# netsniff-ng/netsniff-ng

Hardware: AMD Instinct MI355X
Metric: Mpkt/s + GB/s device-resident dissect, 64B & IMIX; bit-exact fields vs ref (higher is better)
Workload: dtype u8

## Files before the change

netsniff-ng_amd/csrc/nsd_internal.h:

```cpp
#ifndef NSD_INTERNAL_H
#define NSD_INTERNAL_H

#include <hip/hip_runtime_api.h>
#include <stddef.h>
#include <stdint.h>
#include <stdio.h>

#include <string>
#include <vector>

#include "../../include/netsniff_dissect.h"

#define NSD_HIDDEN __attribute__((visibility("hidden")))

NSD_HIDDEN inline bool hip_ok(hipError_t e, const char *what)
{
	if (e != hipSuccess) {
		fprintf(stderr, "netsniff-dissect: %s: %s\n", what, hipGetErrorString(e));
		return false;
	}
	return true;
}

template <class T>
NSD_HIDDEN inline bool grow(T *&p, size_t &cap, size_t need)
{
	if (need <= cap)
		return true;
	if (p)
		(void)hipFree(p);
	p = nullptr;
	cap = 0;
	const size_t want = need + need / 4 + 64;
	if (!hip_ok(hipMalloc(&p, want * sizeof(T)), "hipMalloc"))
		return false;
	cap = want;
	return true;
}

inline size_t batch_extent(const nsd_desc_t *desc, size_t n)
{
	size_t used = 0;
	for (size_t j = 0; j < n; j++) {
		const size_t e = NSD_DESC_OFF(desc[j]) + NSD_DESC_CAPLEN(desc[j]);
		used = e > used ? e : used;
	}
	return used;
}

extern "C" int nsd_launch_dissect_rec(const uint8_t *d_frames, const uint64_t *d_desc, const void *d_sll,
				      uint32_t n, int start_id, int mode, void *d_rec, int compact, uint32_t *d_ext,
				      uint32_t ext_words, uint32_t *d_ext_used, uint64_t *d_counters, void *d_ws,
				      int grid, hipStream_t stream);
extern "C" int nsd_launch_dissect(const uint8_t *d_frames, const uint64_t *d_desc, uint32_t n, int start_id,
				  int mode, nsd_rec *d_rec, uint32_t *d_ext, uint32_t ext_words, uint32_t *d_ext_used,
				  uint64_t *d_counters, void *d_ws, int grid, hipStream_t stream);
extern "C" int nsd_launch_dissect_sll(const uint8_t *d_frames, const uint64_t *d_desc, const void *d_sll,
				      uint32_t n, int start_id, int mode, nsd_rec *d_rec, uint32_t *d_ext,
				      uint32_t ext_words, uint32_t *d_ext_used, uint64_t *d_counters, void *d_ws,
				      int grid, hipStream_t stream);
extern "C" size_t nsd_launch_workspace_bytes(uint32_t n);

NSD_HIDDEN int nsd_start_for(int linktype);
extern "C" NSD_HIDDEN int nsd_pipe_retarget(nsd_pipe *p, int linktype, int mode);

extern "C" NSD_HIDDEN long nsd_flow_feed_host(nsd_flow_table *t, const uint8_t *frames, size_t frames_len,
					      const nsd_desc_t *desc, const nsd_sll_t *sll, uint32_t n, int linktype,
					      int mode, const nsd_bpf_prog *filter, const uint64_t *ts, uint64_t *ts_max,
					      uint64_t base);
extern "C" NSD_HIDDEN int nsd_flow_feed_records(nsd_flow_table *t, const uint8_t *frames, size_t frames_len,
						const nsd_desc_t *desc, uint32_t n, const nsd_rec *rec,
						const uint32_t *ext, uint32_t ext_words, const uint64_t *ts, uint64_t base);
NSD_HIDDEN long nsd_flow_expire_rows(nsd_flow_table *t, uint64_t before, uint32_t flags, uint32_t max,
				     std::vector<nsd_flow> &rows, uint64_t *stats);
NSD_HIDDEN long nsd_flow_expire_rows_ts(nsd_flow_table *t, uint64_t before_ns, uint32_t flags, uint32_t max,
					std::vector<nsd_flowt> &rows, uint64_t *stats);

extern "C" NSD_HIDDEN void nsd_if_cache_reset(void);
extern "C" NSD_HIDDEN void nsd_replay_release(void);
extern "C" NSD_HIDDEN void nsd_device_ctx_release(void);

namespace nsd {
bool render_layer(std::string &s, const uint8_t *pkt, uint32_t caplen, int id, uint32_t start, uint32_t tail,
		  int mode, uint16_t ip_csum, bool icmp_bad, const nsd_sll_t *sll, uint32_t &data,
		  uint32_t &ntail, bool &next);
void render_hex(std::string &s, const uint8_t *pkt, uint32_t caplen, uint32_t from, uint32_t len);
void render_ascii(std::string &s, const uint8_t *pkt, uint32_t caplen, uint32_t from, uint32_t len);
void format_frame_hdr(std::string &s, const nsd_frame_hdr_t &fh, const nsd_sll_t *sll, const uint8_t *pkt,
		      uint32_t caplen, int linktype, int mode, uint64_t count);
int render_packet_cpu(std::string &text, const uint8_t *packet, size_t len, int linktype, int mode,
		      const nsd_sll_t *sll);
int format_replay_part(std::string &s, const uint8_t *frames, const nsd_desc_t *desc, const nsd_frame_hdr_t *fh,
		       const nsd_sll_t *sll, const nsd_crec *rec, const uint32_t *ext, uint64_t count0, uint32_t lo,
		       uint32_t hi, int linktype, int mode);
int cpu_step(int mode, const uint8_t *pkt, uint32_t caplen, int id, uint32_t &data, uint32_t &tail,
	     uint16_t &ip_csum, uint8_t &flags, const nsd_sll_t *sll);
void cpu_count_packet(const uint8_t *pkt, uint32_t caplen, int linktype, int mode, const nsd_sll_t *sll,
		      uint64_t *counters);
}

#endif
```

netsniff-ng_amd/csrc/nsd_kernels.hip:

```cpp
#include <hip/hip_runtime.h>
#include <stdint.h>
#include <string.h>

#include <atomic>
#include <mutex>

#include "nsd_internal.h"
#include "nsd_walk.h"

namespace nsd {

constexpr int BLOCK = 256;
constexpr int WAVES = BLOCK / 64;

#ifndef NSD_WIN2
#define NSD_WIN2 128
#endif
#ifndef NSD_CSUM_U
#define NSD_CSUM_U 12
#endif
#ifndef NSD_FAST_CSUM_U
#define NSD_FAST_CSUM_U 8
#endif
#ifndef NSD_CSUM_LANES
#define NSD_CSUM_LANES 8
#endif
#ifndef NSD_MINW
#define NSD_MINW 4
#endif
#ifndef NSD_FAST_MINW
#define NSD_FAST_MINW 4
#endif
#ifndef NSD_FAST_MINW_FULL
#define NSD_FAST_MINW_FULL 4
#endif
#ifndef NSD_FAST_BPC
#define NSD_FAST_BPC 3
#endif
#ifndef NSD_FAST_BPC_SMALL
#define NSD_FAST_BPC_SMALL 2
#endif
#ifndef NSD_GROUP_BLOCKS
#define NSD_GROUP_BLOCKS 4u
#endif
#ifndef NSD_L2PF
#define NSD_L2PF 16
#endif
#ifndef NSD_REFILL
#define NSD_REFILL 16
#endif
#ifndef NSD_WIN_AHEAD
#define NSD_WIN_AHEAD 32
#endif
#ifndef NSD_SCHED_SAMPLE
#define NSD_SCHED_SAMPLE 32
#endif
#ifndef NSD_SMALL_FRAME
#define NSD_SMALL_FRAME 128
#endif

constexpr int WIN1 = 64;
constexpr int WIN2 = NSD_WIN2;
constexpr int row_of(int W) { return W / 4 + 4; }

typedef uint32_t v4u __attribute__((ext_vector_type(4)));
typedef __attribute__((address_space(1))) const v4u gv4u;
__device__ __forceinline__ uint32_t lanes_below(uint64_t m)
{
	return __builtin_amdgcn_mbcnt_hi((uint32_t)(m >> 32), __builtin_amdgcn_mbcnt_lo((uint32_t)m, 0));
}

__device__ __forceinline__ uint64_t wave_sum64(uint64_t v)
{
#pragma unroll
	for (int o = 32; o > 0; o >>= 1)
		v += __shfl_xor(v, o, 64);
	return v;
}

struct HbmBytes {
	const uint8_t *p;
	uint32_t caplen;
	__device__ __forceinline__ uint8_t b(uint32_t o) const { return o < caplen ? p[o] : 0; }
	__device__ __forceinline__ uint16_t be16(uint32_t o) const { return (uint16_t)(b(o) << 8 | b(o + 1)); }
};

template <bool FAST, int WIN>
struct LSrc {
	const uint32_t *win;
	const uint8_t *lay3t;
	const uint32_t *stept;
	const uint8_t *p;
	uint32_t caplen;
	uint32_t m;
	uint32_t wb;
	mutable bool miss;
	uint32_t sw;
	uint32_t wl = WIN;

	__device__ __forceinline__ uint32_t dw(uint32_t j) const { return win[j ^ sw]; }
	__device__ __forceinline__ int lay3(uint32_t key) const { return lay3t[key & 255]; }
	__device__ __forceinline__ uint32_t step(int id) const { return stept[id & 31]; }
	__device__ __forceinline__ uint32_t l2h(uint32_t h) const { return stept[32 + (h & 31)]; }
	__device__ __forceinline__ uint32_t dword_at(uint32_t o) const
	{
		const uint32_t r = o + m - wb;
		uint32_t j = r >> 2;
		j = j > WIN / 4 - 1 ? WIN / 4 - 1 : j;
		const uint32_t v = __builtin_amdgcn_alignbyte(dw(j + 1), dw(j), r & 3);
		if constexpr (FAST)
			return o >= caplen ? 0u : v;
		return v;
	}
	__device__ __forceinline__ bool missed() const { return miss; }
	__device__ __forceinline__ uint8_t b(uint32_t o) const
	{
		const uint32_t r = o + m - wb;
		if constexpr (FAST) {
			if (r < WIN)
				return (uint8_t)(dw(r >> 2) >> ((r & 3) * 8));
			if (o < caplen)
				miss = true;
			return 0;
		} else {
			if (o >= caplen)
				return 0;
			return r < wl ? (uint8_t)(dw(r >> 2) >> ((r & 3) * 8)) : p[o];
		}
	}
	__device__ __forceinline__ uint16_t le16(uint32_t o) const
	{
		const uint32_t r = o + m - wb;
		if (r + 1 < wl && (r & 3) != 3 && (FAST || o + 2 <= caplen))
			return (uint16_t)(dw(r >> 2) >> ((r & 3) * 8));
		return (uint16_t)(b(o) | b(o + 1) << 8);
	}
	__device__ __forceinline__ uint16_t be16(uint32_t o) const
	{
// ... 1108 lines not shown
constexpr int FROW = WIN1 / 4;

struct FastShared {
	alignas(16) uint32_t win[WAVES][64 * FROW];
	unsigned long long cnt[NSD_NCOUNTERS];
	uint32_t ops[32];
	uint8_t lay3[256];
	uint32_t pcnt[WAVES];
};

__device__ __forceinline__ void stage_write_sw(uint32_t *wwin, const Chunks<WIN1> &ch, int lane)
{
#pragma unroll
	for (int r = 0; r < 4; r++) {
		const int t = r * 64 + lane;
		const int q = t / 4, c = t % 4;
		const uint32_t nv = (ch.nv >> (8 * r)) & 0xFF;
		uint32_t w[4] = { ch.v[r].x, ch.v[r].y, ch.v[r].z, ch.v[r].w };
		if (nv < 16) {
#pragma unroll
			for (int j = 0; j < 4; j++) {
				const uint32_t bp = 4 * j;
				if (bp >= nv)
					w[j] = 0;
				else if (bp + 4 > nv)
					w[j] &= (1u << ((nv - bp) * 8)) - 1u;
			}
		}
		*(uint4 *)(wwin + q * FROW + ((c ^ swz_of((uint32_t)q, 4)) << 2)) = make_uint4(w[0], w[1], w[2], w[3]);
	}
}

__device__ __forceinline__ uint32_t fold_weighted(uint32_t sum, bool odd)
{
	sum = (sum >> 16) + (sum & 0xFFFF);
	sum = (sum >> 16) + (sum & 0xFFFF);
	return odd ? ((sum & 0xFF) << 8 | sum >> 8) : sum;
}

static_assert(k_plain_lay3[6] == NSD_OPS_TCP && k_plain_lay3[17] == NSD_OPS_UDP,
	      "plain_walk's protocol map differs from eth_lay3");

__device__ __forceinline__ bool plain_is(const LSrc<true, WIN1> &s, uint32_t caplen)
{
	const uint32_t r = s.m + 12, j = r >> 2, sh = r & 3;
	const uint32_t d12 = __builtin_amdgcn_alignbyte(s.dw(j + 1), s.dw(j), sh);
	const uint32_t d20 = __builtin_amdgcn_alignbyte(s.dw(j + 3), s.dw(j + 2), sh);
	const uint32_t proto = d20 >> 24;
	return caplen >= 42 && (d12 & 0xFFFFFFu) == 0x450008u && (proto == 6 || proto == 17);
}

__device__ __forceinline__ void plain_walk(const LSrc<true, WIN1> &s, uint32_t caplen, WalkOut &w)
{
	const uint32_t r = s.m + 12, j = r >> 2, sh = r & 3;
	const uint32_t w0 = s.dw(j), w1 = s.dw(j + 1), w2 = s.dw(j + 2), w3 = s.dw(j + 3), w4 = s.dw(j + 4),
		       w5 = s.dw(j + 5), w6 = s.dw(j + 6);
	const uint32_t d12 = __builtin_amdgcn_alignbyte(w1, w0, sh), d16 = __builtin_amdgcn_alignbyte(w2, w1, sh),
		       d20 = __builtin_amdgcn_alignbyte(w3, w2, sh), d24 = __builtin_amdgcn_alignbyte(w4, w3, sh),
		       d28 = __builtin_amdgcn_alignbyte(w5, w4, sh), d32 = __builtin_amdgcn_alignbyte(w6, w5, sh);
	uint32_t sum = (d12 >> 16) + (d32 & 0xFFFF);
	sum = __builtin_amdgcn_sad_u16(d16, 0u, sum);
	sum = __builtin_amdgcn_sad_u16(d20, 0u, sum);
	sum = __builtin_amdgcn_sad_u16(d24, 0u, sum);
	sum = __builtin_amdgcn_sad_u16(d28, 0u, sum);
	sum = (sum >> 16) + (sum & 0xffff);
	sum += sum >> 16;
	w.ip_csum = (uint16_t)~sum;
	const int32_t x = (int32_t)__builtin_bswap16((uint16_t)d16) - 20;
	if (x >= 0 && (uint32_t)x < caplen - 34)
		w.tail = 34 + (uint32_t)x;
	const bool tcp = (d20 >> 24) == 6;
	const int l4 = tcp ? NSD_OPS_TCP : NSD_OPS_UDP;
	w.chain = NSD_OPS_ETHERNET | NSD_OPS_IPV4 << 5 | (uint32_t)l4 << 10;
	w.offA = (uint64_t)14 << 16 | (uint64_t)34 << 32;
	w.n = 3;
	const uint32_t len = w.tail - 34, hl = tcp ? 20u : 8u;
	w.data = len >= hl ? 34 + hl : 34;
}

template <int MODE, bool CR>
__device__ __forceinline__ void fast_tiles(FastShared &sh, const uint8_t *__restrict__ frames,
					   const uint64_t *__restrict__ desc, uint32_t n, int start_id,
					   void *__restrict__ rec, const uint32_t *__restrict__ sll, uint32_t *__restrict__ side,
					   uint4 *__restrict__ list, uint32_t cap, uint32_t &ndef, uint32_t &nicmp)
{
	constexpr int SW = 2;
	const int lane = threadIdx.x & 63;
	const int wv = threadIdx.x >> 6;
	const uint32_t stride = gridDim.x * BLOCK;
	FlagCnt fc;
	uint32_t base = blockIdx.x * BLOCK + wv * 64;

	if (MODE != PRINT_NORM && MODE != PRINT_LESS) {
		for (; base < n; base += stride) {
			const uint32_t i = base + lane;
			fc.pkts += FlagCnt::pc(i < n);
			if (i < n) {
				const uint32_t caplen = NSD_DESC_CAPLEN(desc[i]);
				if constexpr (CR)
					__builtin_nontemporal_store(v2u{ 0u, 0u }, (v2u *)rec + i);
				else
					store_rec((uint4 *)rec, i, make_uint4(0, caplen << 16, 0, 0));
				fc.bytes += caplen;
			}
		}
		fc.flush(sh.cnt, lane);
		return;
	}
	if (base >= n)
		return;
	uint32_t *const rows = &sh.win[wv][0];
	auto dsc = [&](uint32_t b) -> uint64_t {
		return desc[b < n && b + lane < n ? b + lane : n - 1];
	};
	auto tile = [&](Chunks<WIN1> &ch, const uint64_t d0, const uint64_t dpre) {
		const uint32_t i = base + lane;
		const bool valid = i < n;
		const uint64_t off = NSD_DESC_OFF(d0);
		const uint32_t caplen = NSD_DESC_CAPLEN(d0);
		WalkOut w;
		walk_init(w, caplen, valid ? start_id : 0);
		stage_write_sw(rows, ch, lane);
		stage_load<WIN1, true>(ch, frames, dpre, lane);
		wave_sync_lds();
		uint32_t fw = FW_DONE;
		const LSrc<true, WIN1> src{ rows + lane * FROW, sh.lay3, nullptr, frames + off, caplen,
					    (uint32_t)off & 15, 0, false, swz_of((uint32_t)lane, 4) << 2 };
		const bool plain = MODE == PRINT_NORM && start_id == NSD_OPS_ETHERNET &&
				   __ballot(valid && !plain_is(src, caplen)) == 0;
		if (plain) {
			if (valid)
				plain_walk(src, caplen, w);
		} else if (valid) {
			fw = fast_walk<MODE, true>(src, caplen, w);
		}
		const bool deferred = fw != FW_DONE;
		wave_sync_lds();
		const bool done = valid && !deferred;
		if (plain) {
			const uint64_t vm = __ballot(valid), tm = __ballot(valid && w.chain >> 10 == NSD_OPS_TCP);
			const uint32_t nv = (uint32_t)__popcll(vm), nt = (uint32_t)__popcll(tm);
			if (lane == 0) {
				atomicAdd(&sh.ops[NSD_OPS_ETHERNET], nv);
				atomicAdd(&sh.ops[NSD_OPS_IPV4], nv);
				if (nt)
					atomicAdd(&sh.ops[NSD_OPS_TCP], nt);
				if (nv - nt)
					atomicAdd(&sh.ops[NSD_OPS_UDP], nv - nt);
			}
			if (valid)
				put_rec_st<CR>(rec, i, w);
			fc.pkts += nv;
			fc.ipbad += FlagCnt::pc(valid && w.ip_csum != 0);
			fc.trim += FlagCnt::pc(valid && w.tail < caplen);
			if (valid)
				fc.bytes += caplen;
			return;
		}
		if (MODE == PRINT_NORM) {
			const bool pnd = w.icmp_pend && done;
			const uint64_t pm = __ballot(pnd);
			if (pnd) {
				const uint32_t part = fold_weighted(w.icmp_sum, ((uint32_t)off + w.icmp_off) & 1);
				uint4 *e = list + (size_t)(cap - 1 - (nicmp + lanes_below(pm))) * SW;
				st_b128(e, make_uint4(i, w.icmp_off | w.icmp_len << 16, part, 0));
				st_b128(e + 1, make_uint4((uint32_t)d0, (uint32_t)(d0 >> 32), 0, 0));
			}
			nicmp += (uint32_t)__popcll(pm);
		}
		{
			uint32_t key = done ? w.chain : 0xFFFFFFFFu;
			for (int it = 0;; it++) {
				const uint64_t pm = __ballot(key != 0xFFFFFFFFu);
				if (!pm)
					break;
				if (it == 2) {
					if (key != 0xFFFFFFFFu)
						for (uint32_t k = 0; k < w.n; k++)
							atomicAdd(&sh.ops[(key >> (5 * k)) & 31], 1u);
					break;
				}
				const int leader = __ffsll((unsigned long long)pm) - 1;
				const uint32_t lk = __shfl(key, leader, 64);
				const uint64_t m = __ballot(key == lk);
				if (lane == leader) {
					const uint32_t cnt = (uint32_t)__popcll(m);
					for (uint32_t k = 0, nl = w.n; k < nl; k++)
						atomicAdd(&sh.ops[(lk >> (5 * k)) & 31], cnt);
				}
				if (key == lk)
					key = 0xFFFFFFFFu;
			}
		}
		if (CR && side && done && (w.flags & NSD_F_HOST)) {
			st_b32(side + i, w.data);
			w.flags |= NSD_F_LEAF_END;
		}
		if (done)
			put_rec_st<CR>(rec, i, w);
		fc.add(w, caplen, done);
		const uint64_t dm = __ballot(deferred);
		if (dm) {
			if (deferred) {
				if (fw == FW_RESTART) {
					walk_init(w, caplen, start_id);
					if (start_id == NSD_OPS_SLL) {
						const uint32_t w0 = sll ? sll[5 * (size_t)i] : 0u;
						const uint32_t w2 = sll ? sll[5 * (size_t)i + 2] : 0u;
						const uint32_t proto = __builtin_bswap16((uint16_t)(w0 >> 16));
						w.chain = NSD_OPS_SLL;
						w.n = 1;
						atomicAdd(&sh.ops[NSD_OPS_SLL], 1u);
						w.id = sll_next(w2 & 0xFFFF, proto, MODE, c_lay2h.e[NSD_L2H(proto)]);
					}
				} else {
					for (uint32_t k = 0; k < w.n; k++)
						atomicAdd(&sh.ops[(w.chain >> (5 * k)) & 31], 1u);
				}
				uint4 *e = list + (size_t)(ndef + lanes_below(dm)) * SW;
				st_b128(e, make_uint4(i, w.data | w.tail << 16,
						      (uint32_t)w.ip_csum | (uint32_t)w.flags << 16 | w.n << 24 |
							      (uint32_t)w.id << 27,
						      w.chain));
				const uint32_t offs = CR ? 0u
							 : ((uint32_t)(w.offA >> 16) & 0xFF) | ((uint32_t)(w.offA >> 32) & 0xFF) << 8 |
								   ((uint32_t)(w.offA >> 48) & 0xFF) << 16 | (w.offB & 0xFF) << 24;
				st_b128(e + 1, make_uint4((uint32_t)d0, (uint32_t)(d0 >> 32), offs, 0));
			}
			ndef += (uint32_t)__popcll(dm);
		}
	};
	uint64_t d0 = dsc(base), d1 = dsc(base + stride), d2 = dsc(base + 2 * stride);
	Chunks<WIN1> chA, chB;
	stage_load<WIN1, true>(chA, frames, d0, lane);
	stage_load<WIN1, true>(chB, frames, d1, lane);
	for (;;) {
		uint64_t d3 = dsc(base + 3 * stride);
		tile(chA, d0, d2);
		d0 = d1;
		d1 = d2;
		d2 = d3;
		base += stride;
		if (base >= n)
			break;
		d3 = dsc(base + 3 * stride);
		tile(chB, d0, d2);
		d0 = d1;
		d1 = d2;
		d2 = d3;
		base += stride;
		if (base >= n)
			break;
	}
	drain_stores();
	fc.flush(sh.cnt, lane);
}

template <int U, bool CR>
__device__ __forceinline__ void fast_icmp_pass(FastShared &sh, const uint8_t *__restrict__ frames,
					       const uint64_t *__restrict__ desc, void *__restrict__ rec,
					       const uint4 *__restrict__ lists, uint32_t cap)
{
	constexpr int SW = 2;
	const int lane = threadIdx.x & 63;
	const int wv = threadIdx.x >> 6;
	const uint32_t sub = lane & 3, grp = lane >> 2;
	uint32_t bad = 0;
	for (int l = 0; l < WAVES; l++) {
		const uint32_t cnt = sh.pcnt[l];
		const uint4 *list = lists + ((size_t)blockIdx.x * WAVES + l) * cap * SW;
		for (uint32_t k0 = 64 * ((wv + l) % WAVES); k0 < cnt; k0 += 64 * WAVES) {
			const bool on = k0 + lane < cnt;
			const uint4 *ep = list + (size_t)(cap - 1 - (k0 + lane)) * SW;
			const uint4 e = on ? ep[0] : make_uint4(0, 0, 0, 0);
			const uint32_t i = e.x;
			const uint64_t a = (on ? NSD_DESC_OFF((uint64_t)ep[1].y << 32 | ep[1].x) : 0) + (e.y & 0xFFFF);
			const uint32_t nb = e.y >> 16;
			for (uint32_t q = 0; q < 64 && k0 + q < cnt; q += 16) {
				const int src = (int)(q + grp);
				const uint32_t alo = __shfl((uint32_t)a, src, 64);
				const uint32_t ahi = __shfl((uint32_t)(a >> 32), src, 64);
				const uint32_t mnb = __shfl(nb, src, 64);
				const uint32_t part = __shfl(e.z, src, 64);
				const bool mon = k0 + (uint32_t)src < cnt;
				const uint32_t s0 = alo & 15, endb = s0 + mnb;
				const uint32_t nch = mon ? (endb + 15) >> 4 : 0u;
				const uint4 *base = (const uint4 *)(frames + ((((uint64_t)ahi << 32) | alo) & ~15ull));
				uint32_t sum = sub == 0 ? part : 0u;
				const uint32_t je = sub == 0 ? 0u : nch - 1;
				if ((sub == 0 && nch > 0) || (sub == 1 && nch > 1))
					sum += csum_chunk(base[je], 16 * je, s0, endb);
				for (uint32_t j = 1 + sub; __ballot(j + 1 < nch); j += 4 * U) {
					uint4 v[U];
#pragma unroll
					for (int u = 0; u < U; u++) {
						const uint32_t jj = j + 4 * u;
						v[u] = jj + 1 < nch ? base[jj] : make_uint4(0, 0, 0, 0);
					}
#pragma unroll
					for (int u = 0; u < U; u++) {
						sum = sum_halves(v[u].x, sum);
						sum = sum_halves(v[u].y, sum);
						sum = sum_halves(v[u].z, sum);
						sum = sum_halves(v[u].w, sum);
					}
				}
				sum = (sum >> 16) + (sum & 0xffff);
				sum += __shfl_xor(sum, 1, 64);
				sum += __shfl_xor(sum, 2, 64);
				const uint32_t mi = __shfl(i, src, 64);
				const bool isbad = mon && sub == 0 && csum_final(sum) != 0;
				if (isbad) {
					uint8_t *nf = (uint8_t *)rec + nflags_at<CR>(mi);
					*nf = *nf | NSD_F_ICMP_BAD;
				}
				bad += FlagCnt::pc(isbad);
			}
		}
	}
	if (lane == 0 && bad)
		atomicAdd(&sh.cnt[NSD_CNT_ICMP_BAD], (unsigned long long)bad);
}

template <int MODE, bool CR>
__device__ __forceinline__ void walk_lists(Shared &sh, uint32_t *s_touch, const uint8_t *__restrict__ frames,
					   const uint64_t *__restrict__ desc, uint32_t n, void *__restrict__ rec,
					   uint32_t *__restrict__ ext, uint32_t ext_words, uint32_t *__restrict__ ext_used,
					   uint32_t chunk, unsigned long long *__restrict__ counters,
					   const uint4 *__restrict__ list, uint32_t cnt, uint64_t *__restrict__ pend,
					   uint32_t region)
{
	constexpr int SW = 2;
	if (threadIdx.x < 64)
		sh.step[threadIdx.x] = threadIdx.x < 32 ? c_step[threadIdx.x] : c_lay2h.e[threadIdx.x - 32];
	if (threadIdx.x < 32)
		sh.ops[threadIdx.x] = 0;
	if (threadIdx.x < 2 * WAVES)
// ... 11 lines not shown
	wk.d = 0;
	wk.i = 0;
	wk.wb = 0;
	wk.wl = 0;
	wk.have = false;
	wk.stage = false;
	WalkOut pw;
	walk_init(pw, 0, 0);
	RingSt rs;
	rs.init();

	auto load = [&](uint32_t k0, uint4 &x0, uint4 &x1) {
		x0 = x1 = make_uint4(0, 0, 0, 0);
		if (k0 + lane < cnt) {
			const uint4 *e = list + (size_t)(k0 + lane) * SW;
			x0 = e[0];
			x1 = e[1];
		}
	};
	uint4 c0, c1, n0, n1;
	load(0, c0, c1);
	load(64, n0, n1);
	for (uint32_t k0 = 0; k0 < cnt; k0 += 64) {
		{
			const uint64_t d = (uint64_t)n1.y << 32 | n1.x;
			const uint32_t m = (uint32_t)NSD_DESC_OFF(d) & 15, caplen = NSD_DESC_CAPLEN(d);
			const uint32_t wb = ((n0.y & 0xFFFF) + m) & ~15u;
			const bool on = k0 + 64 + lane < cnt && wb < caplen + m;
			const uint64_t a = (uint64_t)frames + (NSD_DESC_OFF(d) & ~15ull) + wb;
			const bool two = on && (a & 127) != 0 && wb + (128 - (uint32_t)(a & 127)) < caplen + m;
			if (on)
				__builtin_amdgcn_global_load_lds((const void *)(a & ~127ull),
								 (__attribute__((address_space(3))) void *)s_touch, 4, 0, 0);
			if (two)
				__builtin_amdgcn_global_load_lds((const void *)((a & ~127ull) + 128),
								 (__attribute__((address_space(3))) void *)s_touch, 4, 0, 0);
		}
		uint4 m0, m1;
		load(k0 + 128, m0, m1);
		bool pnd = k0 + lane < cnt;
		const uint32_t pi = c0.x;
		const uint64_t pd = (uint64_t)c1.y << 32 | c1.x;
		walk_init(pw, c0.y >> 16, (int)(c0.z >> 27));
		pw.data = c0.y & 0xFFFF;
		pw.ip_csum = (uint16_t)c0.z;
		pw.flags = (uint8_t)(c0.z >> 16);
		pw.n = (c0.z >> 24) & 7;
		pw.chain = c0.w;
		if (!CR) {
			pw.offA = (uint64_t)(c1.z & 0xFF) << 16 | (uint64_t)((c1.z >> 8) & 0xFF) << 32 |
				  (uint64_t)((c1.z >> 16) & 0xFF) << 48;
			pw.offB = c1.z >> 24;
		}
		walkers<MODE, CR, false>(sh, rs, frames, rec, g, pq, fc, wk, pnd, pw, pi, pd, false);
		c0 = n0;
		c1 = n1;
		n0 = m0;
		n1 = m1;
	}
	{
		bool none = false;
		if (__ballot(wk.have))
			walkers<MODE, CR, false>(sh, rs, frames, rec, g, pq, fc, wk, none, pw, 0, 0, true);
	}
	fc.flush(sh.cnt, lane);
	leaf_pass<MODE, CR>(frames, desc, rec, ext, pq);
	if (lane == 0)
		sh.pcnt[wv] = pq.npend;
	if (MODE == PRINT_NORM) {
		__syncthreads();
		icmp_pass<NSD_CSUM_U, CR>(sh, frames, desc, rec, pend, region);
	}
	block_flush(sh.cnt, counters);
	if (threadIdx.x < 32 && sh.ops[threadIdx.x])
		atomicAdd(&counters[NSD_CNT_OPS + threadIdx.x], (unsigned long long)sh.ops[threadIdx.x]);
}

template <int MODE, bool CR>
__global__ __launch_bounds__(BLOCK, CR ? NSD_FAST_MINW : NSD_FAST_MINW_FULL) void dissect_fast(
	const uint8_t *__restrict__ frames, const uint64_t *__restrict__ desc, uint32_t n, int start_id,
	void *__restrict__ rec, unsigned long long *__restrict__ counters, uint4 *__restrict__ lists, uint32_t cap,
	const uint32_t *__restrict__ sll, uint32_t *__restrict__ side, unsigned long long *__restrict__ sched,
	uint32_t *__restrict__ ext, uint32_t ext_words, uint32_t *__restrict__ ext_used, uint32_t chunk,
	uint64_t *__restrict__ pend, uint32_t region)
{
	constexpr int SW = 2;
	union FastLds {
		FastShared f;
		Shared w;
	};
	__shared__ FastLds su;
	FastShared &sh = su.f;
	if (threadIdx.x < 32)
		sh.ops[threadIdx.x] = 0;
	block_init(sh.cnt, sh.lay3);
	const int lane = threadIdx.x & 63, wv = threadIdx.x >> 6;
	const uint32_t gw = blockIdx.x * WAVES + wv;
	uint4 *const list = lists + (size_t)gw * cap * SW;
	uint32_t ndef = 0, nicmp = 0;
	fast_tiles<MODE, CR>(sh, frames, desc, n, start_id, rec, sll, side, list, cap, ndef, nicmp);
	if (lane == 0) {
		sh.pcnt[wv] = nicmp;
		if (sched && ndef)
			atomicAdd(&sched[0], (unsigned long long)ndef);
		if (sched && nicmp)
			atomicAdd(&sched[1], (unsigned long long)nicmp);
	}
	if (MODE == PRINT_NORM) {
		__syncthreads();
		fast_icmp_pass<NSD_FAST_CSUM_U, CR>(sh, frames, desc, rec, lists, cap);
	}
	block_flush(sh.cnt, counters);
	if (threadIdx.x < 32 && sh.ops[threadIdx.x])
		atomicAdd(&counters[NSD_CNT_OPS + threadIdx.x], (unsigned long long)sh.ops[threadIdx.x]);
	if constexpr (MODE == PRINT_NORM || MODE == PRINT_LESS) {
		if (__syncthreads_or(ndef != 0)) {
			__shared__ uint32_t s_touch[64];
			walk_lists<MODE, CR>(su.w, s_touch, frames, desc, n, rec, ext, ext_words, ext_used, chunk, counters,
					     list, min(ndef, cap), pend, region);
		}
	}
}

}

constexpr uint32_t NSD_MAX_GRID = 4096;

static uint32_t region_for(uint32_t n, uint32_t blocks)
{
	const uint64_t stride = (uint64_t)blocks * nsd::BLOCK;
	return (uint32_t)(((n + stride - 1) / stride) * nsd::BLOCK);
}
static uint32_t region_for_fused(uint32_t n, uint32_t blocks, bool compact)
{
	return compact ? 2 * region_for(n, blocks) + nsd::WAVES * 4 * 64 : region_for(n, blocks);
}

static size_t region_slots(uint32_t n)
{
	return ((size_t)n + (size_t)NSD_MAX_GRID * nsd::BLOCK + 1) & ~(size_t)1;
}

namespace {
constexpr int MAX_DEV = 16;
struct Sched {
	bool init = false, fused = false, pending = false, small = false;
	bool walky = false;
	bool sampled_once = false;
	bool recorded = false;
	bool discard = false;
	int launches = 0, last = 0;
	uint64_t sampled = 0;
	unsigned long long *host = nullptr;
	hipEvent_t ev = nullptr;
	int cus = 0;
};
Sched g_sched[MAX_DEV];
std::mutex g_sched_mu;
int g_sched_force = 0;
int g_ring_force = 0;
std::atomic<int> g_grid_cap{ 0 };
std::atomic<int> g_debug_fill{ -1 };

int cur_dev()
{
	int d = 0;
	if (hipGetDevice(&d) != hipSuccess || d < 0 || d >= MAX_DEV)
		d = 0;
	return d;
}

struct Plan {
	bool fused, sample, small, prio, ring;
	int cus;
};
Plan sched_plan(uint32_t n, unsigned long long *pair, const uint64_t *counters, hipStream_t stream)
{
	std::lock_guard<std::mutex> g(g_sched_mu);
	const int dev = cur_dev();
	Sched &S = g_sched[dev];
	if (!S.cus) {
		int cus = 0;
		if (hipDeviceGetAttribute(&cus, hipDeviceAttributeMultiprocessorCount, dev) != hipSuccess || cus < 1)
			cus = 256;
		S.cus = cus;
	}
	Plan p{ false, false, false, true, true, S.cus };
	hipStreamCaptureStatus cs = hipStreamCaptureStatusNone;
	const bool capturing = hipStreamIsCapturing(stream, &cs) == hipSuccess && cs != hipStreamCaptureStatusNone;
	const bool landed = !capturing && S.pending && S.recorded && hipEventQuery(S.ev) == hipSuccess;
	if (landed && S.discard) {
		S.pending = S.recorded = S.discard = false;
	} else if (landed) {
		const double rd = S.sampled ? (double)S.host[0] / (double)S.sampled : 0.0;
		const double ri = S.sampled ? (double)S.host[1] / (double)S.sampled : 0.0;
		S.fused = S.fused ? rd > 0.05 || ri > 0.05 : rd > 0.15 || ri > 0.10;
		const uint64_t pk = S.host[4] - S.host[2], by = S.host[5] - S.host[3];
		if (pk)
			S.small = by <= (uint64_t)NSD_SMALL_FRAME * pk;
		S.walky = rd > 0.25;
		S.sampled_once = true;
		S.pending = false;
		S.recorded = false;
	}
	if (!S.init && !capturing) {
		S.init = true;
		if (hipHostMalloc((void **)&S.host, 64, hipHostMallocDefault) != hipSuccess ||
		    hipEventCreateWithFlags(&S.ev, hipEventDisableTiming) != hipSuccess)
			S.host = nullptr;
	}
	p.fused = g_sched_force ? g_sched_force == NSD_SCHED_FUSED : S.fused;
	p.small = S.small;
	p.prio = !S.walky;
	p.ring = g_ring_force ? g_ring_force == 1 : !S.sampled_once || S.walky;
	if (!capturing && ++S.launches >= NSD_SCHED_SAMPLE && !S.pending && S.host && pair && counters &&
	    hipMemsetAsync(pair, 0, 16, stream) == hipSuccess &&
	    hipMemcpyAsync(S.host + 2, counters + NSD_CNT_PKTS, 16, hipMemcpyDeviceToHost, stream) == hipSuccess) {
		p.sample = true;
		S.launches = 0;
		S.sampled = n;
		S.pending = true;
		S.recorded = false;
	}
	S.last = p.fused ? NSD_SCHED_FUSED : NSD_SCHED_SPLIT;
	return p;
}

void sched_fail(Sched &S, hipStream_t stream)
{
	S.discard = true;
	if (hipEventRecord(S.ev, stream) == hipSuccess) {
		S.recorded = true;
		return;
	}
	(void)hipStreamSynchronize(stream);
	S.pending = S.recorded = S.discard = false;
}

void sched_sampled(unsigned long long *pair, const uint64_t *counters, hipStream_t stream)
{
	std::lock_guard<std::mutex> g(g_sched_mu);
	Sched &S = g_sched[cur_dev()];
	if (hipMemcpyAsync(S.host, pair, 16, hipMemcpyDeviceToHost, stream) != hipSuccess ||
	    hipMemcpyAsync(S.host + 4, counters + NSD_CNT_PKTS, 16, hipMemcpyDeviceToHost, stream) != hipSuccess ||
	    hipEventRecord(S.ev, stream) != hipSuccess) {
		sched_fail(S, stream);
		return;
	}
	S.recorded = true;
}

void sched_abort(hipStream_t stream)
{
	std::lock_guard<std::mutex> g(g_sched_mu);
	sched_fail(g_sched[cur_dev()], stream);
}
}

extern "C" int nsd_set_schedule(int sched)
{
	if (sched != NSD_SCHED_ADAPTIVE && sched != NSD_SCHED_SPLIT && sched != NSD_SCHED_FUSED)
		return NSD_ERR_ARG;
	std::lock_guard<std::mutex> g(g_sched_mu);
	const int prev = g_sched_force;
	g_sched_force = sched;
	return prev;
}

extern "C" int nsd_set_record_ring(int mode)
{
	if (mode < 0 || mode > 2)
		return NSD_ERR_ARG;
	std::lock_guard<std::mutex> g(g_sched_mu);
	const int prev = g_ring_force;
	g_ring_force = mode;
	return prev;
}

extern "C" int nsd_set_grid_cap(int blocks)
{
	if (blocks < 0)
		return NSD_ERR_ARG;
	return g_grid_cap.exchange(blocks);
}

extern "C" int nsd_set_debug_fill(int byte)
{
	if (byte < -1 || byte > 255)
		return NSD_ERR_ARG;
	return g_debug_fill.exchange(byte);
}

extern "C" int nsd_last_schedule(void)
{
	std::lock_guard<std::mutex> g(g_sched_mu);
	return g_sched[cur_dev()].last;
}

static size_t align256(size_t x) { return (x + 255) & ~(size_t)255; }
static size_t gtiles_at(uint32_t n)
{
	const size_t slots = region_slots(n);
	return align256(align256(32 * slots) + align256((size_t)NSD_MAX_GRID * nsd::WAVES * 8) + 16 * slots);
}
static size_t sched_pair_at(uint32_t n)
{
	return gtiles_at(n) + (size_t)NSD_MAX_GRID * 128;
}
extern "C" size_t nsd_launch_workspace_bytes(uint32_t n)
{
	return sched_pair_at(n) + 256;
}

extern "C" int nsd_launch_dissect(const uint8_t *d_frames, const uint64_t *d_desc, uint32_t n,
				  int start_id, int mode, nsd_rec *d_rec, uint32_t *d_ext,
				  uint32_t ext_words, uint32_t *d_ext_used, uint64_t *d_counters,
				  void *d_ws, int grid, hipStream_t stream)
{
	return nsd_launch_dissect_rec(d_frames, d_desc, nullptr, n, start_id, mode, d_rec, 0, d_ext, ext_words,
				      d_ext_used, d_counters, d_ws, grid, stream);
}

extern "C" int nsd_launch_dissect_sll(const uint8_t *d_frames, const uint64_t *d_desc, const void *d_sll,
				      uint32_t n, int start_id, int mode, nsd_rec *d_rec, uint32_t *d_ext,
				      uint32_t ext_words, uint32_t *d_ext_used, uint64_t *d_counters,
				      void *d_ws, int grid, hipStream_t stream)
{
	return nsd_launch_dissect_rec(d_frames, d_desc, d_sll, n, start_id, mode, d_rec, 0, d_ext, ext_words,
				      d_ext_used, d_counters, d_ws, grid, stream);
}

extern "C" int nsd_launch_dissect_rec(const uint8_t *d_frames, const uint64_t *d_desc, const void *d_sll,
				      uint32_t n, int start_id, int mode, void *d_rec, int compact, uint32_t *d_ext,
				      uint32_t ext_words, uint32_t *d_ext_used, uint64_t *d_counters, void *d_ws,
				      int grid, hipStream_t stream)
{
	using namespace nsd;
	if (n == 0)
		return 0;
	const int mi = mode == PRINT_NORM ? 0 : mode == PRINT_LESS ? 1 : 2;
	const int ci = compact ? 1 : 0;
	const uint32_t waves = (n + 63) / 64;
	const uint32_t want = (waves + WAVES - 1) / WAVES;
	if (ext_words > NSD_EXT_POOL_MAX_WORDS)
		ext_words = NSD_EXT_POOL_MAX_WORDS;
	auto chunk_for = [&](uint32_t blocks) {
		const uint64_t per = (uint64_t)ext_words / (2ull * blocks * WAVES);
		const uint32_t lo = NSD_EXT_WORDS(NSD_EXT_MAX_LAYERS), hi = 512 * NSD_EXT_WORDS(16);
		return (uint32_t)(per < lo ? lo : per > hi ? hi : per) & ~3u;
	};
	auto occupancy = [&](const void *f, std::atomic<int> &slot, int dflt) {
		int occ = slot.load(std::memory_order_relaxed);
		if (!occ) {
			if (hipOccupancyMaxActiveBlocksPerMultiprocessor(&occ, f, BLOCK, 0) != hipSuccess || occ < 1)
				occ = dflt;
			slot.store(occ, std::memory_order_relaxed);
		}
		return occ;
	};
	if (grid <= 0)
		grid = g_grid_cap.load(std::memory_order_relaxed);
	const int fill = g_debug_fill.load(std::memory_order_relaxed);
	if (fill >= 0) {
		hipStreamCaptureStatus cs = hipStreamCaptureStatusNone;
		if (hipStreamIsCapturing(stream, &cs) == hipSuccess && cs == hipStreamCaptureStatusNone) {
			if (hipMemsetAsync(d_rec, fill, (size_t)n * (compact ? sizeof(nsd_crec) : sizeof(nsd_rec)), stream) != hipSuccess ||
			    (d_ext && ext_words && hipMemsetAsync(d_ext, fill, (size_t)ext_words * 4, stream) != hipSuccess) ||
			    (d_ws && hipMemsetAsync(d_ws, fill, nsd_launch_workspace_bytes(n), stream) != hipSuccess))
				return -2;
		}
	}
	unsigned long long *const pair = d_ws ? (unsigned long long *)((uint8_t *)d_ws + sched_pair_at(n)) : nullptr;
	const Plan plan = sched_plan(n, mi != 2 ? pair : nullptr, d_counters, stream);
	const int s_cus = plan.cus;
	unsigned long long *const sched = plan.sample ? pair : nullptr;
	auto launched = [&]() {
		if (hipGetLastError() == hipSuccess)
			return true;
		if (sched)
			sched_abort(stream);
		return false;
	};
	if (mi != 2 && plan.fused) {
		typedef void (*kfn)(const uint8_t *, const uint64_t *, uint32_t, int, void *, uint32_t *, uint32_t,
				    uint32_t *, uint32_t, unsigned long long *, uint64_t *, uint32_t, const uint32_t *,
				    unsigned long long *, uint32_t *, uint32_t);
		static const kfn kernels[2][3] = {
			{ dissect_all<PRINT_NORM, false>, dissect_all<PRINT_LESS, false>, dissect_all<PRINT_HEX, false> },
			{ dissect_all<PRINT_NORM, true>, dissect_all<PRINT_LESS, true>, dissect_all<PRINT_HEX, true> },
		};
		static const kfn ring_kernels[2] = { dissect_all<PRINT_NORM, true, true>,
						     dissect_all<PRINT_LESS, true, true> };
		static std::atomic<int> s_occ[2][3], s_rocc[2];
		const bool ring = plan.ring && ci == 1 && mi < 2;
		const kfn f = ring ? ring_kernels[mi] : kernels[ci][mi];
		std::atomic<int> &occ_slot = ring ? s_rocc[mi] : s_occ[ci][mi];
		uint32_t cap_blocks = grid > 0 ? (uint32_t)grid
					       : (uint32_t)(s_cus * occupancy((const void *)f, occ_slot, 4));
		if (cap_blocks > NSD_MAX_GRID)
			cap_blocks = NSD_MAX_GRID;
		const uint32_t blocks = want < cap_blocks ? want : cap_blocks;
		uint32_t *const gtiles = (uint32_t *)((uint8_t *)d_ws + gtiles_at(n));
		if (compact) {
			hipLaunchKernelGGL(zero_tiles, dim3((blocks + 255) / 256), dim3(256), 0, stream, gtiles, blocks);
			if (!launched())
				return -2;
		}
		hipLaunchKernelGGL(f, dim3(blocks), dim3(BLOCK), 0, stream, d_frames, d_desc, n, start_id, d_rec, d_ext,
				   ext_words, d_ext_used, chunk_for(blocks), (unsigned long long *)d_counters,
				   (uint64_t *)d_ws, region_for_fused(n, blocks, compact), (const uint32_t *)d_sll, sched,
				   gtiles, plan.prio ? 1u : 0u);
	} else {
		typedef void (*ffn)(const uint8_t *, const uint64_t *, uint32_t, int, void *, unsigned long long *, uint4 *,
				    uint32_t, const uint32_t *, uint32_t *, unsigned long long *, uint32_t *, uint32_t,
				    uint32_t *, uint32_t, uint64_t *, uint32_t);
		static const ffn fast[2][3] = {
			{ dissect_fast<PRINT_NORM, false>, dissect_fast<PRINT_LESS, false>, dissect_fast<PRINT_HEX, false> },
			{ dissect_fast<PRINT_NORM, true>, dissect_fast<PRINT_LESS, true>, dissect_fast<PRINT_HEX, true> },
		};
		static std::atomic<int> s_focc[2][3];
		uint32_t fcap = grid > 0 ? (uint32_t)grid
					 : (uint32_t)(s_cus * occupancy((const void *)fast[ci][mi], s_focc[ci][mi], 8));
		const int bpc = plan.small ? NSD_FAST_BPC_SMALL : NSD_FAST_BPC;
		if (grid <= 0 && bpc > 0 && fcap > (uint32_t)(s_cus * bpc))
			fcap = (uint32_t)(s_cus * bpc);
		if (fcap > NSD_MAX_GRID)
			fcap = NSD_MAX_GRID;
		const uint32_t fblocks = want < fcap ? want : fcap;
		const uint32_t cap = region_for(n, fblocks) / WAVES;
		const uint32_t nlists = fblocks * WAVES;
		const size_t slotb = 32;
		uint8_t *ws = (uint8_t *)d_ws;
		uint4 *lists = (uint4 *)ws;
		uint64_t *pend = (uint64_t *)(ws + align256(slotb * nlists * cap) + align256((size_t)nlists * 8));
		uint32_t *side = compact && d_ext && ext_words >= n ? d_ext : nullptr;
		hipLaunchKernelGGL(fast[ci][mi], dim3(fblocks), dim3(BLOCK), 0, stream, d_frames, d_desc, n, start_id,
				   d_rec, (unsigned long long *)d_counters, lists, cap, (const uint32_t *)d_sll, side, sched,
				   d_ext, ext_words, d_ext_used, chunk_for(fblocks), pend, cap * WAVES);
	}
	if (!launched())
		return -2;
	if (sched)
		sched_sampled(sched, d_counters, stream);
	return 0;
}
```

Measured before the change: 83040.

## Add dynamic tail work-stealing via atomic head counters in fast dissect kernel

```diff
diff --git a/netsniff-ng_amd/csrc/nsd_internal.h b/netsniff-ng_amd/csrc/nsd_internal.h
--- a/netsniff-ng_amd/csrc/nsd_internal.h
+++ b/netsniff-ng_amd/csrc/nsd_internal.h
@@ -60,6 +60,8 @@
 				      uint32_t ext_words, uint32_t *d_ext_used, uint64_t *d_counters, void *d_ws,
 				      int grid, hipStream_t stream);
 extern "C" size_t nsd_launch_workspace_bytes(uint32_t n);
+extern "C" int nsd_launch_workspace_layout(uint32_t n, uint32_t blocks, int compact, uint64_t *out);
+extern "C" int nsd_last_tail_shared(void);
 
 NSD_HIDDEN int nsd_start_for(int linktype);
 extern "C" NSD_HIDDEN int nsd_pipe_retarget(nsd_pipe *p, int linktype, int mode);
diff --git a/netsniff-ng_amd/csrc/nsd_kernels.hip b/netsniff-ng_amd/csrc/nsd_kernels.hip
--- a/netsniff-ng_amd/csrc/nsd_kernels.hip
+++ b/netsniff-ng_amd/csrc/nsd_kernels.hip
@@ -54,6 +54,18 @@
 #endif
 #ifndef NSD_SCHED_SAMPLE
 #define NSD_SCHED_SAMPLE 32
+#endif
+#ifndef NSD_TAIL_DIV
+#define NSD_TAIL_DIV 2
+#endif
+#ifndef NSD_TAIL_MIN_ROUNDS
+#define NSD_TAIL_MIN_ROUNDS 16
+#endif
+#ifndef NSD_TAIL_HEAD_BLOCKS
+#define NSD_TAIL_HEAD_BLOCKS 16
+#endif
+#ifndef NSD_TAIL_TRIES
+#define NSD_TAIL_TRIES 3u
 #endif
 #ifndef NSD_SMALL_FRAME
 #define NSD_SMALL_FRAME 128
@@ -1328,14 +1340,16 @@
 __device__ __forceinline__ void fast_tiles(FastShared &sh, const uint8_t *__restrict__ frames,
 					   const uint64_t *__restrict__ desc, uint32_t n, int start_id,
 					   void *__restrict__ rec, const uint32_t *__restrict__ sll, uint32_t *__restrict__ side,
-					   uint4 *__restrict__ list, uint32_t cap, uint32_t &ndef, uint32_t &nicmp)
+					   uint4 *__restrict__ list, uint32_t cap, uint32_t &ndef, uint32_t &nicmp,
+					   uint32_t *__restrict__ heads, uint32_t tail0, uint32_t nheads)
 {
 	constexpr int SW = 2;
 	const int lane = threadIdx.x & 63;
-	const int wv = threadIdx.x >> 6;
+	const int wv = __builtin_amdgcn_readfirstlane((int)(threadIdx.x >> 6));
 	const uint32_t stride = gridDim.x * BLOCK;
 	FlagCnt fc;
-	uint32_t base = blockIdx.x * BLOCK + wv * 64;
+	auto uni = [](uint32_t x) -> uint32_t { return (uint32_t)__builtin_amdgcn_readfirstlane((int)x); };
+	uint32_t base = uni(blockIdx.x * BLOCK + wv * 64);
 
 	if (MODE != PRINT_NORM && MODE != PRINT_LESS) {
 		for (; base < n; base += stride) {
@@ -1412,7 +1426,7 @@
 				st_b128(e, make_uint4(i, w.icmp_off | w.icmp_len << 16, part, 0));
 				st_b128(e + 1, make_uint4((uint32_t)d0, (uint32_t)(d0 >> 32), 0, 0));
 			}
-			nicmp += (uint32_t)__popcll(pm);
+			nicmp = uni(nicmp + (uint32_t)__popcll(pm));
 		}
 		{
 			uint32_t key = done ? w.chain : 0xFFFFFFFFu;
@@ -1473,32 +1487,110 @@
 								   ((uint32_t)(w.offA >> 48) & 0xFF) << 16 | (w.offB & 0xFF) << 24;
 				st_b128(e + 1, make_uint4((uint32_t)d0, (uint32_t)(d0 >> 32), offs, 0));
 			}
-			ndef += (uint32_t)__popcll(dm);
+			ndef = uni(ndef + (uint32_t)__popcll(dm));
 		}
 	};
-	uint64_t d0 = dsc(base), d1 = dsc(base + stride), d2 = dsc(base + 2 * stride);
+	const uint32_t ntiles = (n + 63) / 64;
+	const uint32_t slim = heads ? tail0 * 64 : n;
+	uint32_t cur = heads ? blockIdx.x % nheads : 0, tries = nheads > 1 ? 0 : NSD_TAIL_TRIES;
+	bool more = heads != nullptr, asked = false;
+	uint32_t gv = 0;
+	auto draw = [&]() {
+		if (lane == 0) {
+			uint32_t z;
+			asm volatile("v_mov_b32 %0, 0" : "=v"(z));
+			gv = atomicAdd(heads + 32 * cur + z, 1u);
+		}
+	};
+	auto ask = [&]() {
+		asked = more && ndef + nicmp + 64u * 7 <= cap;
+		more = asked;
+		if (asked)
+			draw();
+	};
+	uint32_t second = n;
+	auto take = [&]() -> uint32_t {
+		if (!asked)
+			return n;
+		asked = false;
+		auto tile_of = [&]() -> uint32_t {
+			const uint32_t k = (uint32_t)__builtin_amdgcn_readfirstlane((int)gv);
+			return tail0 + 2 * (cur + k * nheads);
+		};
+		uint32_t t = tile_of();
+		auto next = [&]() {
+			tries++;
+			cur = cur + 1 == nheads ? 0 : cur + 1;
+			draw();
+			t = tile_of();
+		};
+		static_assert(NSD_TAIL_TRIES == 3, "take(): one nested test per try");
+		if (t >= ntiles && tries < NSD_TAIL_TRIES) {
+			next();
+			if (t >= ntiles && tries < NSD_TAIL_TRIES) {
+				next();
+				if (t >= ntiles && tries < NSD_TAIL_TRIES)
+					next();
+			}
+		}
+		if (t >= ntiles) {
+			more = false;
+			return n;
+		}
+		second = t + 1 < ntiles ? (t + 1) * 64 : n;
+		if (second == n)
+			more = false;
+		return t * 64;
+	};
+	uint32_t nxt = uni(base + 3 * stride);
+	auto step = [&]() -> uint32_t {
+		uint32_t b;
+		if (nxt < slim) {
+			b = nxt;
+			nxt = uni(nxt + stride);
+			if (nxt >= slim)
+				ask();
+		} else if (second < n) {
+			b = second;
+			second = n;
+		} else {
+			b = take();
+			ask();
+		}
+		return b;
+	};
+	uint32_t b1 = base + stride < slim ? base + stride : n, b2 = base + 2 * stride < slim ? base + 2 * stride : n;
+	uint64_t d0 = dsc(base), d1 = dsc(b1), d2 = dsc(b2);
 	Chunks<WIN1> chA, chB;
 	stage_load<WIN1, true>(chA, frames, d0, lane);
 	stage_load<WIN1, true>(chB, frames, d1, lane);
 	for (;;) {
-		uint64_t d3 = dsc(base + 3 * stride);
+		uint32_t b3 = uni(step());
+		uint64_t d3 = dsc(b3);
 		tile(chA, d0, d2);
 		d0 = d1;
 		d1 = d2;
 		d2 = d3;
-		base += stride;
+		base = uni(b1);
+		b1 = b2;
+		b2 = b3;
 		if (base >= n)
 			break;
-		d3 = dsc(base + 3 * stride);
+		b3 = uni(step());
+		d3 = dsc(b3);
 		tile(chB, d0, d2);
 		d0 = d1;
 		d1 = d2;
 		d2 = d3;
-		base += stride;
+		base = uni(b1);
+		b1 = b2;
+		b2 = b3;
 		if (base >= n)
 			break;
 	}
 	drain_stores();
+	if (lane == 0 && ndef + nicmp > cap)
+		atomicAdd(&sh.cnt[NSD_CNT_LISTOVF], 1ull);
 	fc.flush(sh.cnt, lane);
 }
 
@@ -1676,7 +1768,7 @@
 	void *__restrict__ rec, unsigned long long *__restrict__ counters, uint4 *__restrict__ lists, uint32_t cap,
 	const uint32_t *__restrict__ sll, uint32_t *__restrict__ side, unsigned long long *__restrict__ sched,
 	uint32_t *__restrict__ ext, uint32_t ext_words, uint32_t *__restrict__ ext_used, uint32_t chunk,
-	uint64_t *__restrict__ pend, uint32_t region)
+	uint64_t *__restrict__ pend, uint32_t region, uint32_t *__restrict__ heads, uint32_t tail0, uint32_t nheads)
 {
 	constexpr int SW = 2;
 	union FastLds {
@@ -1692,7 +1784,7 @@
 	const uint32_t gw = blockIdx.x * WAVES + wv;
 	uint4 *const list = lists + (size_t)gw * cap * SW;
 	uint32_t ndef = 0, nicmp = 0;
-	fast_tiles<MODE, CR>(sh, frames, desc, n, start_id, rec, sll, side, list, cap, ndef, nicmp);
+	fast_tiles<MODE, CR>(sh, frames, desc, n, start_id, rec, sll, side, list, cap, ndef, nicmp, heads, tail0, nheads);
 	if (lane == 0) {
 		sh.pcnt[wv] = nicmp;
 		if (sched && ndef)
@@ -1708,7 +1800,12 @@
 	if (threadIdx.x < 32 && sh.ops[threadIdx.x])
 		atomicAdd(&counters[NSD_CNT_OPS + threadIdx.x], (unsigned long long)sh.ops[threadIdx.x]);
 	if constexpr (MODE == PRINT_NORM || MODE == PRINT_LESS) {
-		if (__syncthreads_or(ndef != 0)) {
+		const bool tail = __syncthreads_or(ndef != 0);
+		if (heads && threadIdx.x == 0 && atomicAdd(heads + 32 * nheads, 1u) == gridDim.x - 1) {
+			for (uint32_t h = 0; h <= nheads; h++)
+				atomicExch(heads + 32 * h, 0u);
+		}
+		if (tail) {
 			__shared__ uint32_t s_touch[64];
 			walk_lists<MODE, CR>(su.w, s_touch, frames, desc, n, rec, ext, ext_words, ext_used, chunk, counters,
 					     list, min(ndef, cap), pend, region);
@@ -1744,6 +1841,7 @@
 	bool recorded = false;
 	bool discard = false;
 	int launches = 0, last = 0;
+	bool last_shared = false;
 	uint64_t sampled = 0;
 	unsigned long long *host = nullptr;
 	hipEvent_t ev = nullptr;
@@ -1767,6 +1865,7 @@
 struct Plan {
 	bool fused, sample, small, prio, ring;
 	int cus;
+	bool capturing;
 };
 Plan sched_plan(uint32_t n, unsigned long long *pair, const uint64_t *counters, hipStream_t stream)
 {
@@ -1779,9 +1878,10 @@
 			cus = 256;
 		S.cus = cus;
 	}
-	Plan p{ false, false, false, true, true, S.cus };
+	Plan p{ false, false, false, true, true, S.cus, false };
 	hipStreamCaptureStatus cs = hipStreamCaptureStatusNone;
 	const bool capturing = hipStreamIsCapturing(stream, &cs) == hipSuccess && cs != hipStreamCaptureStatusNone;
+	p.capturing = capturing;
 	const bool landed = !capturing && S.pending && S.recorded && hipEventQuery(S.ev) == hipSuccess;
 	if (landed && S.discard) {
 		S.pending = S.recorded = S.discard = false;
@@ -1820,6 +1920,42 @@
 	return p;
 }
 
+constexpr uint32_t NSD_TAIL_HEADS_MAX = 256;
+constexpr int NSD_TAIL_SETS = 64;
+struct TailSet {
+	int dev;
+	hipStream_t stream;
+	uint32_t *heads;
+};
+TailSet g_tail[NSD_TAIL_SETS];
+int g_ntail = 0;
+
+uint32_t *tail_set(hipStream_t stream)
+{
+	if (stream == hipStreamPerThread)
+		return nullptr;
+	std::lock_guard<std::mutex> g(g_sched_mu);
+	const int dev = cur_dev();
+	for (int k = 0; k < g_ntail; k++)
+		if (g_tail[k].dev == dev && g_tail[k].stream == stream)
+			return g_tail[k].heads;
+	if (g_ntail == NSD_TAIL_SETS)
+		return nullptr;
+	const size_t bytes = (size_t)(NSD_TAIL_HEADS_MAX + 1) * 128;
+	uint32_t *h = nullptr;
+	if (hipMalloc((void **)&h, bytes) != hipSuccess) {
+		(void)hipGetLastError();
+		return nullptr;
+	}
+	if (hipMemsetAsync(h, 0, bytes, stream) != hipSuccess) {
+		(void)hipGetLastError();
+		(void)hipFree(h);
+		return nullptr;
+	}
+	g_tail[g_ntail++] = TailSet{ dev, stream, h };
+	return h;
+}
+
 void sched_fail(Sched &S, hipStream_t stream)
 {
 	S.discard = true;
@@ -1885,6 +2021,12 @@
 	return g_debug_fill.exchange(byte);
 }
 
+extern "C" int nsd_last_tail_shared(void)
+{
+	std::lock_guard<std::mutex> g(g_sched_mu);
+	return g_sched[cur_dev()].last_shared ? 1 : 0;
+}
+
 extern "C" int nsd_last_schedule(void)
 {
 	std::lock_guard<std::mutex> g(g_sched_mu);
@@ -1904,6 +2046,79 @@
 extern "C" size_t nsd_launch_workspace_bytes(uint32_t n)
 {
 	return sched_pair_at(n) + 256;
+}
+
+struct FastCarve {
+	uint32_t rounds, cap;
+	size_t lists_bytes, pend_at, pend_bytes;
+	bool ok;
+};
+static FastCarve fast_carve(uint32_t n, uint32_t fblocks, bool shared)
+{
+	FastCarve c;
+	c.rounds = region_for(n, fblocks) / nsd::BLOCK;
+	c.cap = c.rounds * 64;
+	if (shared)
+		c.cap += c.cap / 5;
+	const size_t nlists = (size_t)fblocks * nsd::WAVES;
+	c.lists_bytes = 32 * nlists * c.cap;
+	c.pend_at = align256(c.lists_bytes) + align256(nlists * 8);
+	c.pend_bytes = 8 * nlists * c.cap;
+	c.ok = c.pend_at + c.pend_bytes <= gtiles_at(n);
+	return c;
+}
+static_assert(NSD_TAIL_DIV == 0 || (NSD_TAIL_DIV >= 2 && NSD_TAIL_MIN_ROUNDS >= 16 && NSD_TAIL_HEAD_BLOCKS >= 16),
+	      "fast_tiles: a static front of more than three rounds, and its liveness argument");
+static uint32_t tail_rounds_for(uint32_t rounds)
+{
+	if (NSD_TAIL_DIV == 0 || rounds < NSD_TAIL_MIN_ROUNDS)
+		return 0;
+	uint32_t t = rounds / NSD_TAIL_DIV;
+	if (!t)
+		t = 1;
+	return t + ((rounds - t) & 1);
+}
+static uint32_t tail_heads_for(uint32_t fblocks)
+{
+	uint32_t h = fblocks / NSD_TAIL_HEAD_BLOCKS;
+	if (h >= 8)
+		h &= ~7u;
+	if (h > NSD_TAIL_HEADS_MAX)
+		h = NSD_TAIL_HEADS_MAX & ~7u;
+	return h ? h : 1;
+}
+
+extern "C" int nsd_launch_workspace_layout(uint32_t n, uint32_t blocks, int compact, uint64_t *out)
+{
+	if (!n || !blocks || !out)
+		return NSD_ERR_ARG;
+	const uint32_t want = ((n + 63) / 64 + nsd::WAVES - 1) / nsd::WAVES;
+	if (blocks > NSD_MAX_GRID)
+		blocks = NSD_MAX_GRID;
+	if (blocks > want)
+		blocks = want;
+	const FastCarve st = fast_carve(n, blocks, false), sh = fast_carve(n, blocks, true);
+	out[0] = nsd_launch_workspace_bytes(n);
+	out[1] = 0;
+	out[2] = 8ull * region_for_fused(n, blocks, compact != 0) * blocks;
+	out[3] = gtiles_at(n);
+	out[4] = compact ? 128ull * blocks : 0;
+	out[5] = sched_pair_at(n);
+	out[6] = 16;
+	out[7] = 0;
+	out[8] = st.lists_bytes;
+	out[9] = st.pend_at;
+	out[10] = st.pend_bytes;
+	out[11] = 0;
+	out[12] = sh.lists_bytes;
+	out[13] = sh.pend_at;
+	out[14] = sh.pend_bytes;
+	out[15] = sh.ok;
+	out[16] = st.cap;
+	out[17] = sh.cap;
+	out[18] = sh.ok ? tail_rounds_for(st.rounds) : 0;
+	out[19] = tail_heads_for(blocks);
+	return 0;
 }
 
 extern "C" int nsd_launch_dissect(const uint8_t *d_frames, const uint64_t *d_desc, uint32_t n,
@@ -2000,6 +2215,10 @@
 			if (!launched())
 				return -2;
 		}
+		{
+			std::lock_guard<std::mutex> g(g_sched_mu);
+			g_sched[cur_dev()].last_shared = false;
+		}
 		hipLaunchKernelGGL(f, dim3(blocks), dim3(BLOCK), 0, stream, d_frames, d_desc, n, start_id, d_rec, d_ext,
 				   ext_words, d_ext_used, chunk_for(blocks), (unsigned long long *)d_counters,
 				   (uint64_t *)d_ws, region_for_fused(n, blocks, compact), (const uint32_t *)d_sll, sched,
@@ -2007,7 +2226,7 @@
 	} else {
 		typedef void (*ffn)(const uint8_t *, const uint64_t *, uint32_t, int, void *, unsigned long long *, uint4 *,
 				    uint32_t, const uint32_t *, uint32_t *, unsigned long long *, uint32_t *, uint32_t,
-				    uint32_t *, uint32_t, uint64_t *, uint32_t);
+				    uint32_t *, uint32_t, uint64_t *, uint32_t, uint32_t *, uint32_t, uint32_t);
 		static const ffn fast[2][3] = {
 			{ dissect_fast<PRINT_NORM, false>, dissect_fast<PRINT_LESS, false>, dissect_fast<PRINT_HEX, false> },
 			{ dissect_fast<PRINT_NORM, true>, dissect_fast<PRINT_LESS, true>, dissect_fast<PRINT_HEX, true> },
@@ -2021,16 +2240,25 @@
 		if (fcap > NSD_MAX_GRID)
 			fcap = NSD_MAX_GRID;
 		const uint32_t fblocks = want < fcap ? want : fcap;
-		const uint32_t cap = region_for(n, fblocks) / WAVES;
-		const uint32_t nlists = fblocks * WAVES;
-		const size_t slotb = 32;
+		FastCarve cv = fast_carve(n, fblocks, true);
+		const uint32_t trounds = mi != 2 && !plan.capturing && cv.ok ? tail_rounds_for(cv.rounds) : 0;
+		uint32_t *const heads = trounds ? tail_set(stream) : nullptr;
+		if (!heads)
+			cv = fast_carve(n, fblocks, false);
+		{
+			std::lock_guard<std::mutex> g(g_sched_mu);
+			g_sched[cur_dev()].last_shared = heads != nullptr;
+		}
+		const uint32_t cap = cv.cap;
+		const uint32_t nheads = tail_heads_for(fblocks);
+		const uint32_t tail0 = heads ? (cv.rounds - trounds) * fblocks * WAVES : 0;
 		uint8_t *ws = (uint8_t *)d_ws;
 		uint4 *lists = (uint4 *)ws;
-		uint64_t *pend = (uint64_t *)(ws + align256(slotb * nlists * cap) + align256((size_t)nlists * 8));
+		uint64_t *pend = (uint64_t *)(ws + cv.pend_at);
 		uint32_t *side = compact && d_ext && ext_words >= n ? d_ext : nullptr;
 		hipLaunchKernelGGL(fast[ci][mi], dim3(fblocks), dim3(BLOCK), 0, stream, d_frames, d_desc, n, start_id,
 				   d_rec, (unsigned long long *)d_counters, lists, cap, (const uint32_t *)d_sll, side, sched,
-				   d_ext, ext_words, d_ext_used, chunk_for(fblocks), pend, cap * WAVES);
+				   d_ext, ext_words, d_ext_used, chunk_for(fblocks), pend, cap * WAVES, heads, tail0, nheads);
 	}
 	if (!launched())
 		return -2;
```

After: 84310 (median of 6 runs). +1.5%, better.
